# ishine/ASR-Rescoring

Measured on NVIDIA B200. Metric: N-best PLL hypotheses/sec, higher is better.
Workload: dtype bf16+fp16head

## Files before the change

### asr-rescoring_b200/build.py

```python
from __future__ import annotations

import os
import subprocess
import sys

HERE = os.path.dirname(os.path.abspath(__file__))
CSRC = os.path.join(HERE, "csrc")
LIB = os.path.join(HERE, "libpllb200.so")
ARCH = ["-gencode", "arch=compute_100a,code=sm_100a"]
COMMON = ["-O3", "-std=c++17", "-lineinfo", "-Xcompiler", "-fPIC", "-Xcompiler", "-Wall",
          "--expt-relaxed-constexpr", "-Xptxas", "-v"]
UNITS = {
    "api.cu": [],
    "gemm_tcgen05.cu": [],
    "gemm_ln_tcgen05.cu": [],
    "encoder_kernels.cu": [],
    "train_kernels.cu": [],
    "train_api.cu": [],
    "bertscore_kernels.cu": [],
    "seq2seq_kernels.cu": [],
    "seq2seq_api.cu": [],
    "rescore_kernels.cu": ["-fmad=false", "-prec-div=true", "-prec-sqrt=true"],
}


def _nvcc() -> str:
    for cand in (os.environ.get("NVCC"), "/usr/local/cuda/bin/nvcc", "nvcc"):
        if cand and (os.path.isabs(cand) and os.path.exists(cand) or not os.path.isabs(cand)):
            return cand
    raise RuntimeError("nvcc not found")
# ... 61 lines not shown
```

### asr-rescoring_b200/csrc/api.cu

```cuda
#include <cuda_bf16.h>

#include <nvtx3/nvToolsExt.h>

#include <algorithm>
#include <cstdlib>
#include <cstring>
#include <unordered_map>
#include <vector>

#include "common.h"

namespace pllb {

static thread_local std::string g_last_error;
thread_local int64_t g_launch_counter = 0;

void set_error(const std::string& msg) { g_last_error = msg; }
int fail(int code, const std::string& msg) {
  g_last_error = msg;
  return code;
}

int check_model_shape(const pllb_model_desc& d) {
  if (d.hidden % 256 != 0 || d.hidden < 256 || d.hidden > 1024 || d.num_heads * 64 != d.hidden ||
// ... 71 lines not shown
  g_tmaps.emplace(key, *out);
  return PLLB_OK;
}

}

using namespace pllb;

namespace {

enum GemmKind { G_QKV = 0, G_AO, G_FF1, G_FF2, G_HEAD, G_DEC, G_KINDS };

struct LayerDev {
  __nv_bfloat16 *qkv_w, *ao_w, *ff1_w, *ff2_w;
  float *qkv_b, *ao_b, *ao_g, *ao_be, *ff1_b, *ff2_b, *out_g, *out_be;
};

struct ClsHead {
  const float* w;
  float b;
  float* out;
};

struct NvtxRange {
  explicit NvtxRange(const char* name) { nvtxRangePushA(name); }
  void next(const char* name) { nvtxRangePop(); nvtxRangePushA(name); }
  ~NvtxRange() { nvtxRangePop(); }
};

struct TimedLaunch {
  cudaEvent_t start, stop;
// ... 1 lines not shown
};

}

struct pllb_context {
  pllb_model_desc d{};
  int device = 0;
  int fp16_from = 0;
  bool head_fp16 = false;
  int dt_head = DT_BF16;
  bool lfp16(int l) const { return l >= fp16_from; }
  int ldt(int l) const { return lfp16(l) ? DT_FP16 : DT_BF16; }
  int ldt_ffn2(int l, bool next_fp16) const { return lfp16(l) ? DT_FP16 : (next_fp16 ? DT_BF16_OUT16 : DT_BF16); }
  bool has_head = false;
  bool share_l0 = true;
  int64_t cap_rows = 0, cap_copies = 0, cap_hyps = 0;
  int vocab_pad = 0, tiles_v = 0;
  std::vector<void*> owned;
  int64_t owned_bytes = 0;
  float *word_emb = nullptr, *pos_emb = nullptr, *type_emb = nullptr, *emb_g = nullptr, *emb_b = nullptr;
  std::vector<LayerDev> layers;
  __nv_bfloat16 *head_w = nullptr, *dec_w = nullptr;
  float *head_b = nullptr, *head_g = nullptr, *head_be = nullptr, *dec_b = nullptr;
  float *hidden_f32 = nullptr, *y_f32 = nullptr;
  __nv_bfloat16 *hidden_bf16 = nullptr, *wide = nullptr , *ctx = nullptr;
  CopyPlan plan{};
  __nv_bfloat16 *hg = nullptr, *t_bf16 = nullptr;
  float *t_f32 = nullptr, *hid_c = nullptr, *label_logit = nullptr, *tok_logp = nullptr;
  float2* partials = nullptr;
  int32_t* meta_dev = nullptr;
// ... 79 lines not shown
               int K, int epi, const LseArgs* lse, cudaStream_t s, int dt) {
  const double fl = 2.0 * (double)M * (double)(epi == EPI_LSE && lse ? lse->vocab : N) * (double)K;
  return timed_launch(c, kind, fl, s, [&] { return launch_gemm_tcgen05(A, W, bias, C, M, N, K, epi, lse, dt, s); });
}

int timed_gemm_ln(pllb_context* c, int kind, const void* A, const void* W, const float* bias, const float* g,
                  const float* be, float* hid32, void* hid16, int64_t M, int K, cudaStream_t s, int dt) {
  const int H = c->d.hidden;
  const double fl = 2.0 * (double)M * (double)H * (double)K;
  return timed_launch(c, kind, fl, s,
                      [&] { return launch_gemm_ln(A, W, bias, g, be, c->d.ln_eps, hid32, hid16, M, H, K, dt, s); });
}

int run_chunk(pllb_context* c, const int32_t* tokens, const int32_t* tok_off, const int32_t* copy_base,
              const int32_t* row_base, int32_t n_hyp, int32_t n_copies, int64_t n_rows, int max_T, double* out_pll,
              float* out_tok_logp, int upto_layer, cudaStream_t s, const ClsHead* cls = nullptr,
              float* out_cls = nullptr) {
  const pllb_model_desc& d = c->d;
  const int H = d.hidden, I = d.intermediate;
  NvtxRange r_chunk("pllb chunk");
  NvtxRange r_stage("stage1: masked-copy expansion + embeddings");
  RC(launch_expand_plan(tokens, tok_off, copy_base, row_base, n_hyp, d.vocab, cls != nullptr, c->plan, s));
  const int n_layers = upto_layer < 0 ? d.num_layers : std::min(upto_layer, d.num_layers);
  const int64_t n_unique = 2 * (int64_t)n_copies + 2 * (int64_t)n_hyp;
  const bool share = c->share_l0 && !cls && 2 * n_unique <= n_rows;
  if (share) {
    RC(launch_embed_unique(tokens, tok_off, n_hyp, c->word_emb, c->pos_emb, c->type_emb, c->emb_g, c->emb_b, d.ln_eps,
                           H, d.cls_id, d.sep_id, d.mask_id, d.vocab, c->y_f32, c->ctx, c->lfp16(0), s));
    RC(launch_row_src(c->plan, n_copies, s));
    RC(launch_rowmajor_to_t32(c->y_f32, c->plan.row_src, c->hidden_f32, n_rows, H, s));
  } else {
    RC(launch_embed_ln(tokens, tok_off, c->plan, n_copies, c->word_emb, c->pos_emb, c->type_emb, c->emb_g, c->emb_b,
// ... 3 lines not shown
  const bool prune_last = upto_layer < 0 && n_layers > 0;
  r_stage.next("stage2: encoder");
  for (int l = 0; l < n_layers; ++l) {
    const LayerDev& L = c->layers[l];
    const bool shared_rows = share && l == 0;
    const bool last = prune_last && l == n_layers - 1;
    const bool f16 = c->lfp16(l);
    const int dt = c->ldt(l);
    const int dt_ffn2 = c->ldt_ffn2(l, l + 1 < d.num_layers ? c->lfp16(l + 1) : (cls ? f16 : c->head_fp16));
    if (last && !shared_rows) {
      RC(timed_gemm(c, G_QKV, c->hidden_bf16, L.qkv_w + (size_t)H * H, L.qkv_b + H, c->wide, n_rows, 2 * H, H,
                    EPI_BIAS_BF16, nullptr, s, dt));
      RC(launch_gather_rows_bf16(c->hidden_bf16, c->plan.mask_row, n_copies, H, c->hg, s));
      RC(timed_gemm(c, G_QKV, c->hg, L.qkv_w, L.qkv_b, c->t_bf16, n_copies, H, H, EPI_BIAS_BF16, nullptr, s, dt));
      RC(launch_attention_row(c->t_bf16, c->wide, c->hg, c->plan, n_copies, H, d.num_heads, max_T, f16, s));
    } else {
      RC(timed_gemm(c, G_QKV, shared_rows ? c->ctx : c->hidden_bf16, L.qkv_w, L.qkv_b, c->wide,
                    shared_rows ? n_unique : n_rows, 3 * H, H, EPI_BIAS_BF16, nullptr, s, dt));
      RC(launch_attention(c->wide, c->ctx, c->plan, n_copies, H, d.num_heads, f16, shared_rows, s));
      if (last) RC(launch_gather_rows_bf16(c->ctx, c->plan.mask_row, n_copies, H, c->hg, s));
    }
    if (last) {
      RC(launch_gather_rows_f32(c->hidden_f32, c->plan.mask_row, n_copies, H, c->hid_c, s));
      RC(timed_gemm_ln(c, G_AO, c->hg, L.ao_w, L.ao_b, L.ao_g, L.ao_be, c->hid_c, c->t_bf16, n_copies, H, s, dt));
      RC(timed_gemm(c, G_FF1, c->t_bf16, L.ff1_w, L.ff1_b, c->wide, n_copies, I, H, EPI_BIAS_GELU_BF16, nullptr, s, dt));
      RC(timed_gemm_ln(c, G_FF2, c->wide, L.ff2_w, L.ff2_b, L.out_g, L.out_be, c->hid_c, c->t_bf16, n_copies, I, s, dt_ffn2));
      break;
    }
    RC(timed_gemm_ln(c, G_AO, c->ctx, L.ao_w, L.ao_b, L.ao_g, L.ao_be, c->hidden_f32, c->hidden_bf16, n_rows, H, s, dt));
    RC(timed_gemm(c, G_FF1, c->hidden_bf16, L.ff1_w, L.ff1_b, c->wide, n_rows, I, H, EPI_BIAS_GELU_BF16, nullptr, s, dt));
// ... 9 lines not shown
  RC(timed_gemm(c, G_HEAD, c->t_bf16, c->head_w, c->head_b, c->t_f32, n_copies, H, H, EPI_BIAS_GELU_F32, nullptr, s,
                c->dt_head));
  RC(launch_plain_ln_bf16(c->t_f32, c->hg, c->head_g, c->head_be, d.ln_eps, n_copies, H, c->head_fp16, s));
  LseArgs lse{c->plan.label, c->partials, c->label_logit, d.vocab};
  RC(timed_gemm(c, G_DEC, c->hg, c->dec_w, c->dec_b, nullptr, n_copies, c->vocab_pad, H, EPI_LSE, &lse, s, c->dt_head));
  RC(launch_lse_finish(c->partials, c->label_logit, n_copies, 2 * c->tiles_v, c->tok_logp, s));
  RC(launch_hyp_sum(c->tok_logp, copy_base, n_hyp, out_pll, out_tok_logp, s));
  return PLLB_OK;
}

struct Chunk {
  int32_t hyp_begin, n_hyp, n_copies;
  int64_t n_rows, tok_begin;
  int max_T;
  int64_t meta_off;
};

int ensure_meta(pllb_context* c, int64_t need, cudaStream_t s) {
  if (need <= c->meta_cap) return PLLB_OK;
  PLLB_CUDA(cudaStreamSynchronize(s));
  PLLB_CUDA(cudaDeviceSynchronize());
  if (c->meta_dev) cudaFree(c->meta_dev);
  if (c->meta_host) cudaFreeHost(c->meta_host);
  c->meta_dev = nullptr;
  c->meta_host = nullptr;
  const int64_t cap = need + need / 2 + 1024;
  PLLB_CUDA(cudaMalloc(&c->meta_dev, sizeof(int32_t) * cap));
  PLLB_CUDA(cudaHostAlloc(&c->meta_host, sizeof(int32_t) * cap, cudaHostAllocDefault));
  c->meta_cap = cap;
  return PLLB_OK;
}
// ... 26 lines not shown
  c->meta_pending = true;
  return PLLB_OK;
}

int score_impl(pllb_context* c, const int32_t* hyp_tokens, const int64_t* off, int32_t n_hyp, double* out_pll,
               float* out_tok_logp, int upto_layer, float* out_hidden, cudaStream_t s, const ClsHead* cls = nullptr) {
  if (!c) return fail(PLLB_ERR_INVALID, "null handle");
  if (n_hyp < 0 || (n_hyp > 0 && (!off || !hyp_tokens && off[n_hyp] > off[0])))
    return fail(PLLB_ERR_INVALID, "pllb_score: null argument");
  PLLB_CUDA(cudaSetDevice(c->device));
  const int64_t launches_before = g_launch_counter;
  c->stats.last_gemm_launches = 0;
  c->timed_used = 0;
  std::vector<Chunk> chunks;
  {
    Chunk cur{0, 0, 0, 0, n_hyp > 0 ? off[0] : 0, 0, 0};
    for (int32_t h = 0; h < n_hyp; ++h) {
      const int64_t L = off[h + 1] - off[h];
      if (L < 0) return fail(PLLB_ERR_INVALID, "pllb_score: offsets not monotone");
      if (L + 2 > c->d.max_position)
        return fail(PLLB_ERR_TOO_LONG, "hypothesis " + std::to_string(h) + " has " + std::to_string(L) +
                                           " tokens; max_position_embeddings allows " + std::to_string(c->d.max_position - 2));
      const int64_t rows = cls ? L + 2 : L * (L + 2);
      const int64_t copies = cls ? 1 : L;
      if (rows > c->cap_rows || copies > c->cap_copies)
        return fail(PLLB_ERR_OOM, "a single hypothesis exceeds max_chunk_tokens");
      if (cur.n_hyp > 0 && (cur.n_rows + rows > c->cap_rows || cur.n_copies + copies > c->cap_copies || cur.n_hyp + 1 > c->cap_hyps)) {
        chunks.push_back(cur);
        cur = Chunk{h, 0, 0, 0, off[h], 0, 0};
      }
      cur.n_hyp += 1;
      cur.n_copies += (int32_t)copies;
      cur.n_rows += rows;
      cur.max_T = std::max(cur.max_T, (int)L + 2);
    }
    if (cur.n_hyp > 0) chunks.push_back(cur);
  }
  if (upto_layer >= 0 && !cls && chunks.size() > 1) return fail(PLLB_ERR_OOM, "pllb_debug_hidden: input must fit one chunk");
  int64_t meta_need = 0;
  for (auto& ch : chunks) {
    ch.meta_off = meta_need;
    meta_need += 3 * (int64_t)(ch.n_hyp + 1);
  }
  RC(ensure_meta(c, meta_need, s));
  RC(meta_acquire(c));
  RC(workspace_acquire(c, s));
  for (const auto& ch : chunks) {
    int32_t* tok_off = c->meta_host + ch.meta_off;
    int32_t* copy_base = tok_off + (ch.n_hyp + 1);
    int32_t* row_base = copy_base + (ch.n_hyp + 1);
    int64_t t = 0, cb = 0, rb = 0;
    for (int32_t i = 0; i <= ch.n_hyp; ++i) {
      tok_off[i] = (int32_t)t; copy_base[i] = (int32_t)cb; row_base[i] = (int32_t)rb;
      if (i < ch.n_hyp) {
        const int64_t L = off[ch.hyp_begin + i + 1] - off[ch.hyp_begin + i];
        t += L; cb += cls ? 1 : L; rb += cls ? L + 2 : L * (L + 2);
      }
    }
  }
  RC(meta_upload(c, meta_need, s));
  if (c->timing) {
    if (!c->ev_begin) { PLLB_CUDA(cudaEventCreate(&c->ev_begin)); PLLB_CUDA(cudaEventCreate(&c->ev_end)); }
    PLLB_CUDA(cudaEventRecord(c->ev_begin, s));
  }
  int64_t row0 = 0;
  for (const auto& ch : chunks) {
    const int32_t* tok_off = c->meta_dev + ch.meta_off;
    const int32_t* copy_base = tok_off + (ch.n_hyp + 1);
    const int32_t* row_base = copy_base + (ch.n_hyp + 1);
    RC(run_chunk(c, hyp_tokens + (ch.tok_begin - off[0]), tok_off, copy_base, row_base, ch.n_hyp, ch.n_copies, ch.n_rows,
                 ch.max_T, out_pll ? out_pll + ch.hyp_begin : nullptr,
                 out_tok_logp ? out_tok_logp + (ch.tok_begin - off[0]) : nullptr, upto_layer, s, cls,
                 cls && cls->out ? cls->out + ch.hyp_begin : nullptr));
    if (out_hidden) RC(launch_t32_to_rowmajor(c->hidden_f32, out_hidden + row0 * c->d.hidden, ch.n_rows, c->d.hidden, s));
    row0 += ch.n_rows;
    c->stats.chunks += 1;
    c->stats.hyps_scored += ch.n_hyp;
    c->stats.copies_scored += ch.n_copies;
    c->stats.tokens_expanded += ch.n_rows;
  }
  if (c->timing) { PLLB_CUDA(cudaEventRecord(c->ev_end, s)); c->have_total = true; }
  RC(workspace_release(c, s));
  c->stats.kernel_launches += g_launch_counter - launches_before;
  return PLLB_OK;
}

int ensure_io(pllb_context* c, int64_t bytes) {
  if (bytes <= c->io_cap) return PLLB_OK;
// ... 72 lines not shown
  if (d.operand_dtype < 0 || (d.operand_dtype > 3 && (d.operand_dtype < 16 || d.operand_dtype > 16 + d.num_layers)))
    return fail(PLLB_ERR_INVALID, "unsupported model shape: need num_layers >= 1, hidden in {256,512,768,1024}, "
                                  "head dim 64, intermediate % 256 == 0");
  PLLB_CUDA(cudaSetDevice(device));
  int major = 0;
  PLLB_CUDA(cudaDeviceGetAttribute(&major, cudaDevAttrComputeCapabilityMajor, device));
  if (major != 10) return fail(PLLB_ERR_NO_DEVICE, "device is not sm_100 (B200); libpllb200 has no other code path");
  pllb_context* c = new pllb_context();
  c->d = d;
  c->device = device;
  c->fp16_from = d.operand_dtype == 1 ? 0 : d.operand_dtype == 3 ? d.num_layers / 2
               : d.operand_dtype >= 16 ? d.operand_dtype - 16 : d.num_layers;
  c->head_fp16 = d.operand_dtype >= 1;
  c->dt_head = c->head_fp16 ? DT_FP16 : DT_BF16;
  if (const char* e = getenv("PLLB_SHARE_L0")) c->share_l0 = atoi(e) != 0;
  cudaStream_t s = 0;
  const int H = d.hidden, I = d.intermediate, V = d.vocab;
  int rc = PLLB_OK;
  auto bail = [&](int code) {
    pllb_destroy(c);
    return code;
  };
#define TRY(expr)                  \
  do {                             \
    rc = (expr);                   \
    if (rc) return bail(rc);       \
  } while (0)
  TRY(copy_f32(c, &c->word_emb, w->word_emb, (int64_t)V * H, s));
  TRY(copy_f32(c, &c->pos_emb, w->pos_emb, (int64_t)d.max_position * H, s));
  TRY(copy_f32(c, &c->type_emb, w->type_emb, H, s));
  TRY(copy_f32(c, &c->emb_g, w->emb_ln_g, H, s));
  TRY(copy_f32(c, &c->emb_b, w->emb_ln_b, H, s));
  c->layers.resize(d.num_layers);
  for (int l = 0; l < d.num_layers; ++l) {
    const pllb_layer_weights& lw = w->layers[l];
    LayerDev& L = c->layers[l];
    TRY(dev_alloc(c, &L.qkv_w, (int64_t)3 * H * H));
    TRY(launch_f32_to_bf16(lw.q_w, L.qkv_w, (int64_t)H * H, c->lfp16(l), s));
    TRY(launch_f32_to_bf16(lw.k_w, L.qkv_w + (int64_t)H * H, (int64_t)H * H, c->lfp16(l), s));
    TRY(launch_f32_to_bf16(lw.v_w, L.qkv_w + (int64_t)2 * H * H, (int64_t)H * H, c->lfp16(l), s));
    TRY(dev_alloc(c, &L.qkv_b, 3 * H));
    cudaMemcpyAsync(L.qkv_b, lw.q_b, sizeof(float) * H, cudaMemcpyDeviceToDevice, s);
    cudaMemcpyAsync(L.qkv_b + H, lw.k_b, sizeof(float) * H, cudaMemcpyDeviceToDevice, s);
    cudaMemcpyAsync(L.qkv_b + 2 * H, lw.v_b, sizeof(float) * H, cudaMemcpyDeviceToDevice, s);
    TRY(conv_16(c, &L.ao_w, lw.ao_w, (int64_t)H * H, c->lfp16(l), s));
    TRY(copy_f32(c, &L.ao_b, lw.ao_b, H, s));
    TRY(copy_f32(c, &L.ao_g, lw.ao_ln_g, H, s));
    TRY(copy_f32(c, &L.ao_be, lw.ao_ln_b, H, s));
    TRY(conv_16(c, &L.ff1_w, lw.ff1_w, (int64_t)I * H, c->lfp16(l), s));
    TRY(copy_f32(c, &L.ff1_b, lw.ff1_b, I, s));
    TRY(conv_16(c, &L.ff2_w, lw.ff2_w, (int64_t)H * I, c->lfp16(l), s));
    TRY(copy_f32(c, &L.ff2_b, lw.ff2_b, H, s));
    TRY(copy_f32(c, &L.out_g, lw.out_ln_g, H, s));
    TRY(copy_f32(c, &L.out_be, lw.out_ln_b, H, s));
  }
  c->vocab_pad = (int)align_up(V, 256);
  c->tiles_v = c->vocab_pad / 256;
  c->has_head = w->head_w && w->head_b && w->head_ln_g && w->head_ln_b && w->decoder_w && w->decoder_b;
  if (c->has_head) {
// ... 567 lines not shown
```

### asr-rescoring_b200/csrc/common.h

```cpp
#pragma once
#include <cuda.h>
#include <cuda_runtime.h>
#include <stdint.h>

#include <cstdio>
#include <string>
#include <utility>
#include <vector>

#include "../../include/pllb.h"

namespace pllb {

void set_error(const std::string& msg);
int fail(int code, const std::string& msg);
extern thread_local int64_t g_launch_counter;
__attribute__((visibility("hidden"))) int check_model_shape(const pllb_model_desc& d);

#define PLLB_CUDA(expr)                                                                        \
  do {                                                                                         \
    cudaError_t _e = (expr);                                                                   \
    if (_e != cudaSuccess)                                                                     \
      return ::pllb::fail(PLLB_ERR_CUDA, std::string(#expr) + ": " + cudaGetErrorString(_e));  \
  } while (0)
// ... 74 lines not shown

int launch_expand_plan(const int32_t* tokens, const int32_t* hyp_tok_off, const int32_t* hyp_copy_base,
                       const int32_t* hyp_row_base, int32_t n_hyp, int32_t vocab, bool whole_sequence, CopyPlan plan,
                       cudaStream_t s);
int launch_expand_ids(const int32_t* tokens, const int32_t* hyp_tok_off, CopyPlan plan, int32_t n_copies,
                      int32_t cls_id, int32_t sep_id, int32_t mask_id, int32_t* out_ids, int32_t* out_mask_pos,
                      int32_t* out_labels, cudaStream_t s);
int launch_embed_ln(const int32_t* tokens, const int32_t* hyp_tok_off, CopyPlan plan, int32_t n_copies,
                    const float* word_emb, const float* pos_emb, const float* type_emb, const float* g,
                    const float* b, float eps, int H, int32_t cls_id, int32_t sep_id, int32_t mask_id, int32_t vocab,
                    float* hidden_f32_rowmajor, void* hidden_bf16, bool fp16, cudaStream_t s);
int launch_plain_ln_bf16(const float* x, void* out_bf16, const float* g, const float* b, float eps, int64_t rows,
                         int H, bool fp16, cudaStream_t s);
int launch_attention(const void* qkv_bf16, void* ctx_bf16, CopyPlan plan, int32_t n_copies, int H, int NH, bool fp16,
                     bool shared_rows, cudaStream_t s);
int launch_embed_unique(const int32_t* tokens, const int32_t* hyp_tok_off, int32_t n_hyp, const float* word_emb,
                        const float* pos_emb, const float* type_emb, const float* g, const float* b, float eps, int H,
                        int32_t cls_id, int32_t sep_id, int32_t mask_id, int32_t vocab, float* u_f32, void* u_bf16,
                        bool fp16, cudaStream_t s);
int launch_row_src(CopyPlan plan, int32_t n_copies, cudaStream_t s);
int launch_attention_row(const void* q_bf16, const void* kv_bf16, void* out_bf16, CopyPlan plan, int32_t n_copies, int H,
                         int NH, int max_T, bool fp16, cudaStream_t s);
int launch_gather_rows_bf16(const void* hidden_bf16, const int32_t* rows, int32_t n, int H, void* out,
                            cudaStream_t s);
int launch_gather_rows_f32(const float* src, const int32_t* rows, int32_t n, int H, float* out, cudaStream_t s);
int launch_cls_linear(const float* hid_t32, const float* w, float b, int32_t n, int H, float* out, cudaStream_t s);
int launch_lse_finish(const float2* partials, const float* label_logit, int32_t n_copies, int n_tiles,
                      float* tok_logp, cudaStream_t s);
int launch_hyp_sum(const float* tok_logp, const int32_t* hyp_copy_base, int32_t n_hyp, double* out_pll,
                   float* out_tok_logp, cudaStream_t s);
// ... 65 lines not shown
```

### asr-rescoring_b200/csrc/encoder_kernels.cu

```cuda
#include <cuda_bf16.h>
#include <cuda_fp16.h>

#include "common.h"
#include "ptx.cuh"

namespace pllb {

namespace {

constexpr int WARPS_PER_BLOCK = 8;

__device__ __forceinline__ float warp_sum(float v) {
#pragma unroll
  for (int o = 16; o > 0; o >>= 1) v += __shfl_xor_sync(0xffffffffu, v, o);
  return v;
}
__device__ __forceinline__ float warp_max(float v) {
#pragma unroll
  for (int o = 16; o > 0; o >>= 1) v = fmaxf(v, __shfl_xor_sync(0xffffffffu, v, o));
  return v;
}

template <bool FP16>
__device__ __forceinline__ uint32_t pack16(float lo, float hi) {
// ... 181 lines not shown
          const float* __restrict__ b, float eps, int64_t rows) {
  constexpr int H = 128 * VEC;
  const int64_t row = (int64_t)blockIdx.x * WARPS_PER_BLOCK + (threadIdx.x >> 5);
  const int lane = threadIdx.x & 31;
  if (row >= rows) return;
  const float4* yr = reinterpret_cast<const float4*>(y + row * H);
  float4 x[VEC];
#pragma unroll
  for (int i = 0; i < VEC; ++i) x[i] = yr[lane + 32 * i];
  ln_normalize<VEC>(x, g, b, eps, lane);
  store_row<VEC, FP16>(x, out_bf16 + row * H, lane);
}

constexpr int ATT_WARPS = 8;
constexpr int ATT_VROW = 72;

__device__ __forceinline__ float fast_ex2(float x) {
  float y;
  asm("ex2.approx.ftz.f32 %0, %1;" : "=f"(y) : "f"(x));
  return y;
}

template <bool FP16>
__device__ __forceinline__ void mma_16816(float (&d)[4], const uint32_t (&a)[4], uint32_t b0, uint32_t b1) {
  if constexpr (FP16) {
    asm volatile(
        "mma.sync.aligned.m16n8k16.row.col.f32.f16.f16.f32 {%0,%1,%2,%3}, {%4,%5,%6,%7}, {%8,%9}, {%0,%1,%2,%3};"
        : "+f"(d[0]), "+f"(d[1]), "+f"(d[2]), "+f"(d[3])
        : "r"(a[0]), "r"(a[1]), "r"(a[2]), "r"(a[3]), "r"(b0), "r"(b1));
  } else {
    asm volatile(
        "mma.sync.aligned.m16n8k16.row.col.f32.bf16.bf16.f32 {%0,%1,%2,%3}, {%4,%5,%6,%7}, {%8,%9}, {%0,%1,%2,%3};"
        : "+f"(d[0]), "+f"(d[1]), "+f"(d[2]), "+f"(d[3])
        : "r"(a[0]), "r"(a[1]), "r"(a[2]), "r"(a[3]), "r"(b0), "r"(b1));
  }
}

struct RowDirect {
  size_t start_ld, ld;
  __device__ __forceinline__ size_t operator()(int r) const { return start_ld + (size_t)r * ld; }
};
struct RowShared {
  int ubase, umask, mpos;
  size_t ld;
  __device__ __forceinline__ size_t operator()(int r) const { return (size_t)(r == mpos ? umask : ubase + r) * ld; }
};

template <bool FP16, class RM>
__device__ __forceinline__ void attn_stream(const __nv_bfloat16* __restrict__ base , const RM rm,
                                            __nv_bfloat16* __restrict__ ob, int T, int H, int lane, __nv_bfloat16* vs) {
  const __nv_bfloat16* kb = base + H;
// ... 715 lines not shown
```

### asr-rescoring_b200/csrc/ptx.cuh

```cuda
#pragma once
#include <cuda.h>
#include <cuda_runtime.h>
#include <stdint.h>

namespace pllb {

__device__ __forceinline__ uint32_t smem_u32(const void* p) {
  return static_cast<uint32_t>(__cvta_generic_to_shared(p));
}

__device__ __forceinline__ bool elect_one() {
  uint32_t pred = 0;
  asm volatile(
      "{\n\t.reg .pred P;\n\t"
      "elect.sync _|P, 0xffffffff;\n\t"
      "selp.b32 %0, 1, 0, P;\n\t}\n"
      : "=r"(pred));
  return pred != 0;
}

template <bool FP16>
__device__ __forceinline__ uint32_t pack16x2_sat(float lo, float hi) {
  uint32_t r;
  if constexpr (FP16) asm("cvt.rn.satfinite.f16x2.f32 %0, %1, %2;" : "=r"(r) : "f"(hi), "f"(lo));
// ... 148 lines not shown
}

__device__ __forceinline__ void tmem_ld_32x32b_x32(uint32_t taddr, uint32_t (&r)[32]) {
  asm volatile(
      "tcgen05.ld.sync.aligned.32x32b.x32.b32 "
      "{%0, %1, %2, %3, %4, %5, %6, %7, %8, %9, %10, %11, %12, %13, %14, %15, "
      "%16, %17, %18, %19, %20, %21, %22, %23, %24, %25, %26, %27, %28, %29, %30, %31}, [%32];"
      : "=r"(r[0]), "=r"(r[1]), "=r"(r[2]), "=r"(r[3]), "=r"(r[4]), "=r"(r[5]), "=r"(r[6]), "=r"(r[7]),
        "=r"(r[8]), "=r"(r[9]), "=r"(r[10]), "=r"(r[11]), "=r"(r[12]), "=r"(r[13]), "=r"(r[14]), "=r"(r[15]),
        "=r"(r[16]), "=r"(r[17]), "=r"(r[18]), "=r"(r[19]), "=r"(r[20]), "=r"(r[21]), "=r"(r[22]), "=r"(r[23]),
        "=r"(r[24]), "=r"(r[25]), "=r"(r[26]), "=r"(r[27]), "=r"(r[28]), "=r"(r[29]), "=r"(r[30]), "=r"(r[31])
      : "r"(taddr)
      : "memory");
}

__device__ __forceinline__ float2 ffma2(float2 a, float2 b, float2 c) {
  float2 d;
  asm("{.reg .b64 ra, rb, rc, rd;\n\t"
      "mov.b64 ra, {%2,%3};\n\t mov.b64 rb, {%4,%5};\n\t mov.b64 rc, {%6,%7};\n\t"
      "fma.rn.f32x2 rd, ra, rb, rc;\n\t mov.b64 {%0,%1}, rd;}"
      : "=f"(d.x), "=f"(d.y) : "f"(a.x), "f"(a.y), "f"(b.x), "f"(b.y), "f"(c.x), "f"(c.y));
  return d;
}
__device__ __forceinline__ float2 fmul2(float2 a, float2 b) {
  float2 d;
  asm("{.reg .b64 ra, rb, rd;\n\t"
      "mov.b64 ra, {%2,%3};\n\t mov.b64 rb, {%4,%5};\n\t"
      "mul.rn.f32x2 rd, ra, rb;\n\t mov.b64 {%0,%1}, rd;}"
      : "=f"(d.x), "=f"(d.y) : "f"(a.x), "f"(a.y), "f"(b.x), "f"(b.y));
  return d;
}
__device__ __forceinline__ float2 fadd2(float2 a, float2 b) {
  float2 d;
  asm("{.reg .b64 ra, rb, rd;\n\t"
      "mov.b64 ra, {%2,%3};\n\t mov.b64 rb, {%4,%5};\n\t"
      "add.rn.f32x2 rd, ra, rb;\n\t mov.b64 {%0,%1}, rd;}"
      : "=f"(d.x), "=f"(d.y) : "f"(a.x), "f"(a.y), "f"(b.x), "f"(b.y));
  return d;
}

__device__ __forceinline__ uint64_t make_kmajor_sw128_desc(uint32_t smem_addr) {
  uint64_t d = 0;
  d |= (uint64_t)((smem_addr & 0x3FFFF) >> 4);
  d |= (uint64_t)1 << 16;
  d |= (uint64_t)(1024 >> 4) << 32;
  d |= (uint64_t)1 << 46;
  d |= (uint64_t)2 << 61;
  return d;
}
__host__ __device__ constexpr uint32_t make_idesc_bf16(int M, int N) {
  return (1u << 4) | (1u << 7) | (1u << 10) | ((uint32_t)(N >> 3) << 17) | ((uint32_t)(M >> 4) << 24);
}
__host__ __device__ constexpr uint32_t make_idesc_f16(int M, int N) {
// ... 9 lines not shown
```

Before: 20760.

## Fuse QKV projection GEMM with per-copy attention in a 2-CTA tcgen05 kernel

Adds a new kernel that computes the QKV projection per head on tcgen05 tensor cores (2-CTA clusters, interleaved per-head QKV weights), stages Q/K/V tiles in shared memory and runs flash-style attention with mma.sync directly from them, writing only the context. Masked copies are packed into 128-row runs on the host so each tile holds whole sequences. The path is used when max_T fits a run and padding overhead stays under 15%. This removes the wide QKV buffer round-trip through global memory and a separate attention launch. The cost is extra weight memory for the interleaved copies, padded rows in runs, and heavier epilogue warps.

Result: no change. 20870, median of 6 (+0.6%).

```diff
diff --git a/asr-rescoring_b200/build.py b/asr-rescoring_b200/build.py
--- a/asr-rescoring_b200/build.py
+++ b/asr-rescoring_b200/build.py
@@ -14,6 +14,7 @@
     "api.cu": [],
     "gemm_tcgen05.cu": [],
     "gemm_ln_tcgen05.cu": [],
+    "fused_attention_tcgen05.cu": [],
     "encoder_kernels.cu": [],
     "train_kernels.cu": [],
     "train_api.cu": [],
diff --git a/asr-rescoring_b200/csrc/api.cu b/asr-rescoring_b200/csrc/api.cu
--- a/asr-rescoring_b200/csrc/api.cu
+++ b/asr-rescoring_b200/csrc/api.cu
@@ -109,7 +109,12 @@
 struct LayerDev {
   __nv_bfloat16 *qkv_w, *ao_w, *ff1_w, *ff2_w;
   float *qkv_b, *ao_b, *ao_g, *ao_be, *ff1_b, *ff2_b, *out_g, *out_be;
+  __nv_bfloat16* qkv_wi = nullptr;
+  float* qkv_bi = nullptr;
 };
+
+constexpr double kFuseMaxPadding = 0.15;
+constexpr int kRunRows = 128;
 
 struct ClsHead {
   const float* w;
@@ -141,6 +146,7 @@
   int ldt_ffn2(int l, bool next_fp16) const { return lfp16(l) ? DT_FP16 : (next_fp16 ? DT_BF16_OUT16 : DT_BF16); }
   bool has_head = false;
   bool share_l0 = true;
+  bool fuse_att = true;
   int64_t cap_rows = 0, cap_copies = 0, cap_hyps = 0;
   int vocab_pad = 0, tiles_v = 0;
   std::vector<void*> owned;
@@ -250,8 +256,8 @@
 
 int run_chunk(pllb_context* c, const int32_t* tokens, const int32_t* tok_off, const int32_t* copy_base,
               const int32_t* row_base, int32_t n_hyp, int32_t n_copies, int64_t n_rows, int max_T, double* out_pll,
-              float* out_tok_logp, int upto_layer, cudaStream_t s, const ClsHead* cls = nullptr,
-              float* out_cls = nullptr) {
+              float* out_tok_logp, int upto_layer, cudaStream_t s, const int32_t* run_copy, int32_t n_runs,
+              const ClsHead* cls = nullptr, float* out_cls = nullptr) {
   const pllb_model_desc& d = c->d;
   const int H = d.hidden, I = d.intermediate;
   NvtxRange r_chunk("pllb chunk");
@@ -285,6 +291,11 @@
       RC(launch_gather_rows_bf16(c->hidden_bf16, c->plan.mask_row, n_copies, H, c->hg, s));
       RC(timed_gemm(c, G_QKV, c->hg, L.qkv_w, L.qkv_b, c->t_bf16, n_copies, H, H, EPI_BIAS_BF16, nullptr, s, dt));
       RC(launch_attention_row(c->t_bf16, c->wide, c->hg, c->plan, n_copies, H, d.num_heads, max_T, f16, s));
+    } else if (n_runs > 0 && !shared_rows) {
+      RC(timed_launch(c, G_QKV, 2.0 * (double)n_rows * 3 * H * H, s, [&] {
+        return launch_fused_qkv_attention(c->hidden_bf16, L.qkv_wi, L.qkv_bi, c->ctx, n_rows, H, d.num_heads, run_copy,
+                                          n_runs, c->plan, f16, s);
+      }));
     } else {
       RC(timed_gemm(c, G_QKV, shared_rows ? c->ctx : c->hidden_bf16, L.qkv_w, L.qkv_b, c->wide,
                     shared_rows ? n_unique : n_rows, 3 * H, H, EPI_BIAS_BF16, nullptr, s, dt));
@@ -324,7 +335,26 @@
   int64_t n_rows, tok_begin;
   int max_T;
   int64_t meta_off;
+  int32_t n_runs;
 };
+
+int32_t plan_runs(const int64_t* off, int32_t hyp_begin, int32_t n_hyp, int32_t* run_copy) {
+  int32_t n_runs = 0, copy = 0;
+  int64_t used = kRunRows;
+  for (int32_t h = hyp_begin; h < hyp_begin + n_hyp; ++h) {
+    const int64_t L = off[h + 1] - off[h], T = L + 2;
+    for (int64_t m = 0; m < L; ++m, ++copy) {
+      if (used + T > kRunRows) {
+        if (run_copy) run_copy[n_runs] = copy;
+        ++n_runs;
+        used = 0;
+      }
+      used += T;
+    }
+  }
+  if (run_copy) run_copy[n_runs] = copy;
+  return n_runs;
+}
 
 int ensure_meta(pllb_context* c, int64_t need, cudaStream_t s) {
   if (need <= c->meta_cap) return PLLB_OK;
@@ -381,7 +411,7 @@
   c->timed_used = 0;
   std::vector<Chunk> chunks;
   {
-    Chunk cur{0, 0, 0, 0, n_hyp > 0 ? off[0] : 0, 0, 0};
+    Chunk cur{0, 0, 0, 0, n_hyp > 0 ? off[0] : 0, 0, 0, 0};
     for (int32_t h = 0; h < n_hyp; ++h) {
       const int64_t L = off[h + 1] - off[h];
       if (L < 0) return fail(PLLB_ERR_INVALID, "pllb_score: offsets not monotone");
@@ -394,7 +424,7 @@
         return fail(PLLB_ERR_OOM, "a single hypothesis exceeds max_chunk_tokens");
       if (cur.n_hyp > 0 && (cur.n_rows + rows > c->cap_rows || cur.n_copies + copies > c->cap_copies || cur.n_hyp + 1 > c->cap_hyps)) {
         chunks.push_back(cur);
-        cur = Chunk{h, 0, 0, 0, off[h], 0, 0};
+        cur = Chunk{h, 0, 0, 0, off[h], 0, 0, 0};
       }
       cur.n_hyp += 1;
       cur.n_copies += (int32_t)copies;
@@ -408,6 +438,13 @@
   for (auto& ch : chunks) {
     ch.meta_off = meta_need;
     meta_need += 3 * (int64_t)(ch.n_hyp + 1);
+    if (c->fuse_att && !cls && ch.max_T <= kRunRows && ch.n_copies > 0) {
+      const int32_t n_runs = plan_runs(off, ch.hyp_begin, ch.n_hyp, nullptr);
+      if ((double)n_runs * kRunRows < (1.0 + kFuseMaxPadding) * (double)ch.n_rows) {
+        ch.n_runs = n_runs;
+        meta_need += n_runs + 1;
+      }
+    }
   }
   RC(ensure_meta(c, meta_need, s));
   RC(meta_acquire(c));
@@ -424,6 +461,7 @@
         t += L; cb += cls ? 1 : L; rb += cls ? L + 2 : L * (L + 2);
       }
     }
+    if (ch.n_runs > 0) plan_runs(off, ch.hyp_begin, ch.n_hyp, row_base + (ch.n_hyp + 1));
   }
   RC(meta_upload(c, meta_need, s));
   if (c->timing) {
@@ -437,8 +475,8 @@
     const int32_t* row_base = copy_base + (ch.n_hyp + 1);
     RC(run_chunk(c, hyp_tokens + (ch.tok_begin - off[0]), tok_off, copy_base, row_base, ch.n_hyp, ch.n_copies, ch.n_rows,
                  ch.max_T, out_pll ? out_pll + ch.hyp_begin : nullptr,
-                 out_tok_logp ? out_tok_logp + (ch.tok_begin - off[0]) : nullptr, upto_layer, s, cls,
-                 cls && cls->out ? cls->out + ch.hyp_begin : nullptr));
+                 out_tok_logp ? out_tok_logp + (ch.tok_begin - off[0]) : nullptr, upto_layer, s,
+                 row_base + (ch.n_hyp + 1), ch.n_runs, cls, cls && cls->out ? cls->out + ch.hyp_begin : nullptr));
     if (out_hidden) RC(launch_t32_to_rowmajor(c->hidden_f32, out_hidden + row0 * c->d.hidden, ch.n_rows, c->d.hidden, s));
     row0 += ch.n_rows;
     c->stats.chunks += 1;
@@ -541,6 +579,7 @@
   c->head_fp16 = d.operand_dtype >= 1;
   c->dt_head = c->head_fp16 ? DT_FP16 : DT_BF16;
   if (const char* e = getenv("PLLB_SHARE_L0")) c->share_l0 = atoi(e) != 0;
+  if (const char* e = getenv("PLLB_FUSE_ATT")) c->fuse_att = atoi(e) != 0;
   cudaStream_t s = 0;
   const int H = d.hidden, I = d.intermediate, V = d.vocab;
   int rc = PLLB_OK;
@@ -570,6 +609,18 @@
     cudaMemcpyAsync(L.qkv_b, lw.q_b, sizeof(float) * H, cudaMemcpyDeviceToDevice, s);
     cudaMemcpyAsync(L.qkv_b + H, lw.k_b, sizeof(float) * H, cudaMemcpyDeviceToDevice, s);
     cudaMemcpyAsync(L.qkv_b + 2 * H, lw.v_b, sizeof(float) * H, cudaMemcpyDeviceToDevice, s);
+    if (c->fuse_att) {
+      TRY(dev_alloc(c, &L.qkv_wi, (int64_t)3 * H * H));
+      TRY(dev_alloc(c, &L.qkv_bi, 3 * H));
+      for (int h = 0; h < d.num_heads; ++h)
+        for (int part = 0; part < 3; ++part) {
+          const int64_t src = (int64_t)part * H + h * 64, dst = (int64_t)h * 192 + part * 64;
+          TRY(cudaMemcpyAsync(L.qkv_wi + dst * H, L.qkv_w + src * H, sizeof(__nv_bfloat16) * 64 * H,
+                              cudaMemcpyDeviceToDevice, s) == cudaSuccess ? PLLB_OK : fail(PLLB_ERR_CUDA, "qkv interleave"));
+          TRY(cudaMemcpyAsync(L.qkv_bi + dst, L.qkv_b + src, sizeof(float) * 64, cudaMemcpyDeviceToDevice, s) == cudaSuccess
+                  ? PLLB_OK : fail(PLLB_ERR_CUDA, "qkv interleave"));
+        }
+    }
     TRY(conv_16(c, &L.ao_w, lw.ao_w, (int64_t)H * H, c->lfp16(l), s));
     TRY(copy_f32(c, &L.ao_b, lw.ao_b, H, s));
     TRY(copy_f32(c, &L.ao_g, lw.ao_ln_g, H, s));
diff --git a/asr-rescoring_b200/csrc/common.h b/asr-rescoring_b200/csrc/common.h
--- a/asr-rescoring_b200/csrc/common.h
+++ b/asr-rescoring_b200/csrc/common.h
@@ -112,6 +112,9 @@
                          int H, bool fp16, cudaStream_t s);
 int launch_attention(const void* qkv_bf16, void* ctx_bf16, CopyPlan plan, int32_t n_copies, int H, int NH, bool fp16,
                      bool shared_rows, cudaStream_t s);
+int launch_fused_qkv_attention(const void* A, const void* W_il, const float* bias_il, void* ctx, int64_t rows, int H,
+                               int NH, const int32_t* run_copy, int32_t n_runs, CopyPlan plan, bool fp16,
+                               cudaStream_t stream);
 int launch_embed_unique(const int32_t* tokens, const int32_t* hyp_tok_off, int32_t n_hyp, const float* word_emb,
                         const float* pos_emb, const float* type_emb, const float* g, const float* b, float eps, int H,
                         int32_t cls_id, int32_t sep_id, int32_t mask_id, int32_t vocab, float* u_f32, void* u_bf16,
diff --git a/asr-rescoring_b200/csrc/encoder_kernels.cu b/asr-rescoring_b200/csrc/encoder_kernels.cu
--- a/asr-rescoring_b200/csrc/encoder_kernels.cu
+++ b/asr-rescoring_b200/csrc/encoder_kernels.cu
@@ -219,27 +219,6 @@
 
 constexpr int ATT_WARPS = 8;
 constexpr int ATT_VROW = 72;
-
-__device__ __forceinline__ float fast_ex2(float x) {
-  float y;
-  asm("ex2.approx.ftz.f32 %0, %1;" : "=f"(y) : "f"(x));
-  return y;
-}
-
-template <bool FP16>
-__device__ __forceinline__ void mma_16816(float (&d)[4], const uint32_t (&a)[4], uint32_t b0, uint32_t b1) {
-  if constexpr (FP16) {
-    asm volatile(
-        "mma.sync.aligned.m16n8k16.row.col.f32.f16.f16.f32 {%0,%1,%2,%3}, {%4,%5,%6,%7}, {%8,%9}, {%0,%1,%2,%3};"
-        : "+f"(d[0]), "+f"(d[1]), "+f"(d[2]), "+f"(d[3])
-        : "r"(a[0]), "r"(a[1]), "r"(a[2]), "r"(a[3]), "r"(b0), "r"(b1));
-  } else {
-    asm volatile(
-        "mma.sync.aligned.m16n8k16.row.col.f32.bf16.bf16.f32 {%0,%1,%2,%3}, {%4,%5,%6,%7}, {%8,%9}, {%0,%1,%2,%3};"
-        : "+f"(d[0]), "+f"(d[1]), "+f"(d[2]), "+f"(d[3])
-        : "r"(a[0]), "r"(a[1]), "r"(a[2]), "r"(a[3]), "r"(b0), "r"(b1));
-  }
-}
 
 struct RowDirect {
   size_t start_ld, ld;
diff --git a/asr-rescoring_b200/csrc/fused_attention_tcgen05.cu b/asr-rescoring_b200/csrc/fused_attention_tcgen05.cu
--- /dev/null
+++ b/asr-rescoring_b200/csrc/fused_attention_tcgen05.cu
@@ -0,0 +1,392 @@
+#include <cuda_bf16.h>
+#include <cuda_fp16.h>
+
+#include <algorithm>
+
+#include "common.h"
+#include "ptx.cuh"
+
+namespace pllb {
+
+namespace {
+
+constexpr int FA_BM = 128;
+constexpr int FA_BN = 192;
+constexpr int FA_BK = 64;
+constexpr int FA_UMMA_K = 16;
+constexpr int FA_STAGES = 4;
+constexpr int FA_A_BYTES = FA_BM * FA_BK * 2;
+constexpr int FA_B_BYTES = (FA_BN / 2) * FA_BK * 2;
+constexpr int FA_EPI_WARPS = 14;
+constexpr int FA_STAGE_WARPS = 12;
+constexpr int FA_WARP_COLS = FA_BN / (FA_STAGE_WARPS / 4);
+constexpr int FA_LD_COLS = 32;
+constexpr int FA_THREADS = 32 * (2 + FA_EPI_WARPS);
+static_assert(FA_WARP_COLS % FA_LD_COLS == 0 && 64 % FA_LD_COLS == 0, "staging chunks");
+constexpr int FA_ACC_STRIDE = 256;
+constexpr int FA_TMEM_COLS = 512;
+constexpr int FA_VROW = 72;
+constexpr int FA_SROWS = FA_BM + 16;
+constexpr int FA_MAT_BYTES = FA_SROWS * FA_VROW * 2;
+constexpr int FA_OUT_BYTES = 16 * FA_VROW * 2;
+constexpr int FA_PIPE = FA_STAGES * (FA_A_BYTES + FA_B_BYTES);
+constexpr int FA_SMEM_STAGE = 3 * FA_MAT_BYTES;
+constexpr int FA_SMEM_OUT = FA_EPI_WARPS * FA_OUT_BYTES;
+constexpr int FA_SMEM_BARS = 256;
+constexpr int FA_SMEM_TOTAL = FA_PIPE + FA_SMEM_STAGE + FA_SMEM_OUT + FA_SMEM_BARS + 1024;
+static_assert(FA_SMEM_TOTAL <= 227 * 1024, "shared memory budget");
+
+struct FaParams {
+  const int32_t* run_copy;
+  int32_t n_runs;
+  const int32_t* seq_start;
+  const int32_t* seq_len;
+  const float* bias;
+  __nv_bfloat16* ctx;
+  int H, NH;
+};
+
+__device__ __forceinline__ void epi_bar(int id) {
+  asm volatile("bar.sync %0, %1;" ::"r"(id), "n"(FA_EPI_WARPS * 32) : "memory");
+}
+
+template <bool FP16>
+__device__ __forceinline__ void attend_block(uint32_t q_addr, uint32_t k_addr, uint32_t v_addr, int m0, int T,
+                                             __nv_bfloat16* __restrict__ ob, int H, int lane, uint32_t out_addr,
+                                             const __nv_bfloat16* out_sm) {
+  const int g = lane >> 2, cq = lane & 3;
+  constexpr float kScaleLog2 = 0.125f * 1.4426950408889634f;
+  const int lrow = (lane & 7) + ((lane >> 3) & 1) * 8, lcol8 = ((lane >> 4) & 1) * 8;
+  uint32_t qf[4][4];
+#pragma unroll
+  for (int ks = 0; ks < 4; ++ks) {
+    const uint32_t addr = q_addr + (uint32_t)((m0 + lrow) * FA_VROW + 16 * ks + lcol8) * 2;
+    asm volatile("ldmatrix.sync.aligned.m8n8.x4.shared.b16 {%0,%1,%2,%3}, [%4];"
+                 : "=r"(qf[ks][0]), "=r"(qf[ks][1]), "=r"(qf[ks][2]), "=r"(qf[ks][3]) : "r"(addr));
+  }
+  float mx[2] = {-INFINITY, -INFINITY}, l[2] = {0.f, 0.f};
+  float o[8][4];
+#pragma unroll
+  for (int n = 0; n < 8; ++n) { o[n][0] = o[n][1] = o[n][2] = o[n][3] = 0.f; }
+  for (int k0 = 0; k0 < T; k0 += 16) {
+    float s[2][4];
+#pragma unroll
+    for (int j = 0; j < 2; ++j) {
+      s[j][0] = s[j][1] = s[j][2] = s[j][3] = 0.f;
+      if (j == 1 && k0 + 8 >= T) break;
+#pragma unroll
+      for (int kp = 0; kp < 2; ++kp) {
+        const uint32_t addr = k_addr + (uint32_t)((k0 + 8 * j + (lane & 7)) * FA_VROW + 32 * kp + (lane >> 3) * 8) * 2;
+        uint32_t b0, b1, b2, b3;
+        asm volatile("ldmatrix.sync.aligned.m8n8.x4.shared.b16 {%0,%1,%2,%3}, [%4];"
+                     : "=r"(b0), "=r"(b1), "=r"(b2), "=r"(b3) : "r"(addr));
+        mma_16816<FP16>(s[j], qf[2 * kp], b0, b1);
+        mma_16816<FP16>(s[j], qf[2 * kp + 1], b2, b3);
+      }
+    }
+    float bm[2] = {-INFINITY, -INFINITY};
+    const bool tail = k0 + 16 > T;
+#pragma unroll
+    for (int j = 0; j < 2; ++j) {
+#pragma unroll
+      for (int e = 0; e < 4; ++e) {
+        const int key = k0 + 8 * j + 2 * cq + (e & 1);
+        s[j][e] = (!tail || key < T) ? s[j][e] * kScaleLog2 : -INFINITY;
+        bm[e >> 1] = fmaxf(bm[e >> 1], s[j][e]);
+      }
+    }
+    float corr[2];
+#pragma unroll
+    for (int r = 0; r < 2; ++r) {
+      bm[r] = fmaxf(bm[r], __shfl_xor_sync(0xffffffffu, bm[r], 1));
+      bm[r] = fmaxf(bm[r], __shfl_xor_sync(0xffffffffu, bm[r], 2));
+      const float nm = fmaxf(mx[r], bm[r]);
+      corr[r] = fast_ex2(mx[r] - nm);
+      mx[r] = nm;
+      l[r] *= corr[r];
+    }
+    uint32_t pf[4];
+    {
+      const float p00 = fast_ex2(s[0][0] - mx[0]), p01 = fast_ex2(s[0][1] - mx[0]);
+      const float p02 = fast_ex2(s[0][2] - mx[1]), p03 = fast_ex2(s[0][3] - mx[1]);
+      const float p10 = fast_ex2(s[1][0] - mx[0]), p11 = fast_ex2(s[1][1] - mx[0]);
+      const float p12 = fast_ex2(s[1][2] - mx[1]), p13 = fast_ex2(s[1][3] - mx[1]);
+      l[0] += (p00 + p01) + (p10 + p11);
+      l[1] += (p02 + p03) + (p12 + p13);
+      pf[0] = pack16x2_sat<FP16>(p00, p01); pf[1] = pack16x2_sat<FP16>(p02, p03);
+      pf[2] = pack16x2_sat<FP16>(p10, p11); pf[3] = pack16x2_sat<FP16>(p12, p13);
+    }
+    if (k0 > 0) {
+#pragma unroll
+      for (int n = 0; n < 8; ++n) {
+        o[n][0] *= corr[0]; o[n][1] *= corr[0]; o[n][2] *= corr[1]; o[n][3] *= corr[1];
+      }
+    }
+#pragma unroll
+    for (int n = 0; n < 8; n += 2) {
+      const uint32_t addr = v_addr + (uint32_t)((k0 + lrow) * FA_VROW + 8 * n + lcol8) * 2;
+      uint32_t b0, b1, b2, b3;
+      asm volatile("ldmatrix.sync.aligned.m8n8.x4.trans.shared.b16 {%0,%1,%2,%3}, [%4];"
+                   : "=r"(b0), "=r"(b1), "=r"(b2), "=r"(b3) : "r"(addr));
+      mma_16816<FP16>(o[n], pf, b0, b1);
+      mma_16816<FP16>(o[n + 1], pf, b2, b3);
+    }
+  }
+#pragma unroll
+  for (int r = 0; r < 2; ++r) {
+    l[r] += __shfl_xor_sync(0xffffffffu, l[r], 1);
+    l[r] += __shfl_xor_sync(0xffffffffu, l[r], 2);
+  }
+  const float inv0 = 1.0f / l[0], inv1 = 1.0f / l[1];
+  __syncwarp();
+  {
+    const uint32_t st0 = out_addr + (uint32_t)(g * FA_VROW + 2 * cq) * 2, st1 = st0 + 8 * FA_VROW * 2;
+#pragma unroll
+    for (int n = 0; n < 8; ++n) {
+      asm volatile("st.shared.b32 [%0], %1;" ::"r"(st0 + 16 * n), "r"(pack16x2_sat<FP16>(o[n][0] * inv0, o[n][1] * inv0)) : "memory");
+      asm volatile("st.shared.b32 [%0], %1;" ::"r"(st1 + 16 * n), "r"(pack16x2_sat<FP16>(o[n][2] * inv1, o[n][3] * inv1)) : "memory");
+    }
+  }
+  __syncwarp();
+  {
+    const int r_off = lane >> 3, ch = lane & 7;
+#pragma unroll
+    for (int rr = 0; rr < 16; rr += 4) {
+      const int q = m0 + rr + r_off;
+      if (q < T)
+        *reinterpret_cast<uint4*>(ob + (size_t)q * H + ch * 8) =
+            *reinterpret_cast<const uint4*>(out_sm + (rr + r_off) * FA_VROW + ch * 8);
+    }
+  }
+}
+
+template <bool FP16>
+__global__ void __launch_bounds__(FA_THREADS, 1)
+fused_qkv_attention_kernel(const __grid_constant__ CUtensorMap tmA, const __grid_constant__ CUtensorMap tmB,
+                           const FaParams p) {
+  extern __shared__ uint8_t smem_raw[];
+  const uint32_t smem_base = (smem_u32(smem_raw) + 1023u) & ~1023u;
+  uint8_t* smem_gen = smem_raw + (smem_base - smem_u32(smem_raw));
+  const uint32_t sA = smem_base;
+  const uint32_t sB = smem_base + FA_STAGES * FA_A_BYTES;
+  const uint32_t sQ = smem_base + FA_PIPE;
+  const uint32_t sOut = sQ + FA_SMEM_STAGE;
+  const uint32_t sBar = sOut + FA_SMEM_OUT;
+  const uint32_t bar_full = sBar;
+  const uint32_t bar_empty = sBar + 8 * FA_STAGES;
+  const uint32_t bar_tfull = sBar + 16 * FA_STAGES;
+  const uint32_t bar_tempty = bar_tfull + 16;
+  const uint32_t tmem_slot = bar_tempty + 16;
+  uint32_t* tmem_slot_ptr = reinterpret_cast<uint32_t*>(smem_gen + (tmem_slot - smem_base));
+
+  const int warp = threadIdx.x >> 5;
+  const int lane = threadIdx.x & 31;
+  const int num_kb = p.H / FA_BK;
+  const uint32_t crank = cluster_ctarank();
+  const int unit0 = (int)(blockIdx.x >> 1);
+  const int unit_stride = (int)(gridDim.x >> 1);
+  const int num_tiles = ((p.n_runs + 1) / 2) * p.NH;
+
+  if (warp == 0 && lane == 0) {
+    prefetch_tensormap(&tmA);
+    prefetch_tensormap(&tmB);
+  }
+  if (warp == 1) {
+    if (lane == 0) {
+      for (int s = 0; s < FA_STAGES; ++s) {
+        mbar_init(bar_full + 8 * s, 1);
+        mbar_init(bar_empty + 8 * s, 1);
+      }
+      for (int s = 0; s < 2; ++s) {
+        mbar_init(bar_tfull + 8 * s, 1);
+        mbar_init(bar_tempty + 8 * s, 2 * FA_STAGE_WARPS);
+      }
+      fence_barrier_init();
+    }
+    __syncwarp();
+    tmem_alloc_2cta(tmem_slot, FA_TMEM_COLS);
+    tmem_relinquish_2cta();
+  }
+  if (warp >= 2) {
+    const int t = threadIdx.x - 64;
+    for (int i = t; i < 3 * 16 * FA_VROW / 8; i += FA_EPI_WARPS * 32) {
+      const int mat = i / (16 * FA_VROW / 8), e = i % (16 * FA_VROW / 8);
+      *reinterpret_cast<uint4*>(smem_gen + FA_PIPE + mat * FA_MAT_BYTES + FA_BM * FA_VROW * 2 + e * 16) =
+          make_uint4(0, 0, 0, 0);
+    }
+  }
+  tcgen05_fence_before();
+  __syncthreads();
+  cluster_sync_all();
+  tcgen05_fence_after();
+  const uint32_t tmem_base = *tmem_slot_ptr;
+
+  if (warp == 0) {
+    if (lane == 0) {
+      uint32_t stage = 0, phase = 0;
+      auto first_row = [&](int tile) {
+        const int run = 2 * (tile / p.NH) + (int)crank;
+        return tile < num_tiles && run < p.n_runs ? p.seq_start[p.run_copy[run]] : 0;
+      };
+      int next_row0 = first_row(unit0);
+      for (int tile = unit0; tile < num_tiles; tile += unit_stride) {
+        const int head = tile % p.NH;
+        const int row0 = next_row0;
+        next_row0 = first_row(tile + unit_stride);
+        for (int kb = 0; kb < num_kb; ++kb) {
+          mbar_wait(bar_empty + 8 * stage, phase ^ 1);
+          const uint32_t lead_full = mapa_shared(bar_full + 8 * stage, 0);
+          if (crank == 0) mbar_arrive_expect_tx(bar_full + 8 * stage, 2 * (FA_A_BYTES + FA_B_BYTES));
+          tma_load_2d_2sm(sA + stage * FA_A_BYTES, &tmA, lead_full, kb * FA_BK, row0);
+          tma_load_2d_2sm(sB + stage * FA_B_BYTES, &tmB, lead_full, kb * FA_BK, head * FA_BN + (int)crank * (FA_BN / 2));
+          if (++stage == FA_STAGES) { stage = 0; phase ^= 1; }
+        }
+      }
+    }
+  } else if (warp == 1) {
+    if (lane == 0 && crank == 0) {
+      constexpr uint32_t idesc = make_idesc_16(2 * FA_BM, FA_BN, FP16, FP16);
+      uint32_t stage = 0, phase = 0, acc = 0, acc_phase = 0;
+      for (int tile = unit0; tile < num_tiles; tile += unit_stride) {
+        mbar_wait(bar_tempty + 8 * acc, acc_phase ^ 1);
+        tcgen05_fence_after();
+        const uint32_t d_tmem = tmem_base + acc * FA_ACC_STRIDE;
+        for (int kb = 0; kb < num_kb; ++kb) {
+          mbar_wait(bar_full + 8 * stage, phase);
+          tcgen05_fence_after();
+          const uint32_t a_addr = sA + stage * FA_A_BYTES;
+          const uint32_t b_addr = sB + stage * FA_B_BYTES;
+#pragma unroll
+          for (int k = 0; k < FA_BK / FA_UMMA_K; ++k) {
+            const uint64_t adesc = make_kmajor_sw128_desc(a_addr + k * FA_UMMA_K * 2);
+            const uint64_t bdesc = make_kmajor_sw128_desc(b_addr + k * FA_UMMA_K * 2);
+            tcgen05_mma_bf16_2cta(d_tmem, adesc, bdesc, idesc, (kb | k) != 0 ? 1u : 0u);
+          }
+          tcgen05_commit_2cta_multicast(bar_empty + 8 * stage, (uint16_t)0x3);
+          if (++stage == FA_STAGES) { stage = 0; phase ^= 1; }
+        }
+        tcgen05_commit_2cta_multicast(bar_tfull + 8 * acc, (uint16_t)0x3);
+        acc ^= 1;
+        if (acc == 0) acc_phase ^= 1;
+      }
+    }
+  } else {
+    const int q = warp & 3;
+    const int ew = warp - 2;
+    const int cbase = (ew >> 2) * FA_WARP_COLS;
+    const int srow = q * 32 + lane;
+    const uint32_t out_addr = sOut + ew * FA_OUT_BYTES;
+    const __nv_bfloat16* out_sm = reinterpret_cast<const __nv_bfloat16*>(smem_gen + FA_PIPE + FA_SMEM_STAGE + ew * FA_OUT_BYTES);
+    uint32_t acc = 0, acc_phase = 0;
+    for (int tile = unit0; tile < num_tiles; tile += unit_stride) {
+      const int run = 2 * (tile / p.NH) + (int)crank;
+      const int head = tile % p.NH;
+      int n_cp = 0, st_a = 0, t_a = 0, st_b = 0, t_b = 0;
+      if (run < p.n_runs) {
+        const int c_begin = p.run_copy[run];
+        n_cp = p.run_copy[run + 1] - c_begin;
+        if (lane < n_cp) { st_a = p.seq_start[c_begin + lane]; t_a = p.seq_len[c_begin + lane]; }
+        if (lane + 32 < n_cp) { st_b = p.seq_start[c_begin + 32 + lane]; t_b = p.seq_len[c_begin + 32 + lane]; }
+      }
+      mbar_wait(bar_tfull + 8 * acc, acc_phase);
+      tcgen05_fence_after();
+      epi_bar(1);
+      const uint32_t t_addr = tmem_base + acc * FA_ACC_STRIDE + ((uint32_t)(q * 32) << 16);
+      const float* bias = p.bias + head * FA_BN;
+#pragma unroll
+      for (int ci = 0; ci < (ew < FA_STAGE_WARPS ? FA_WARP_COLS / FA_LD_COLS : 0); ++ci) {
+        const int c0 = cbase + FA_LD_COLS * ci;
+        uint32_t r[FA_LD_COLS];
+        tmem_ld_32x32b_x32(t_addr + c0, r);
+        tcgen05_wait_ld();
+        if (ci == FA_WARP_COLS / FA_LD_COLS - 1) {
+          tcgen05_fence_before();
+          __syncwarp();
+          if (lane == 0) mbar_arrive_cluster(mapa_shared(bar_tempty + 8 * acc, 0));
+        }
+        const uint32_t dst = sQ + (uint32_t)(c0 >> 6) * FA_MAT_BYTES + (uint32_t)(srow * FA_VROW + (c0 & 63)) * 2;
+        const float4* bias4 = reinterpret_cast<const float4*>(bias + c0);
+#pragma unroll
+        for (int c = 0; c < FA_LD_COLS / 8; ++c) {
+          const float4 b0 = __ldg(bias4 + 2 * c), b1 = __ldg(bias4 + 2 * c + 1);
+          const float2 v0 = fadd2(make_float2(__uint_as_float(r[8 * c + 0]), __uint_as_float(r[8 * c + 1])), make_float2(b0.x, b0.y));
+          const float2 v1 = fadd2(make_float2(__uint_as_float(r[8 * c + 2]), __uint_as_float(r[8 * c + 3])), make_float2(b0.z, b0.w));
+          const float2 v2 = fadd2(make_float2(__uint_as_float(r[8 * c + 4]), __uint_as_float(r[8 * c + 5])), make_float2(b1.x, b1.y));
+          const float2 v3 = fadd2(make_float2(__uint_as_float(r[8 * c + 6]), __uint_as_float(r[8 * c + 7])), make_float2(b1.z, b1.w));
+          asm volatile("st.shared.v4.b32 [%0], {%1, %2, %3, %4};" ::"r"(dst + 16 * c),
+                       "r"(pack16x2_sat<FP16>(v0.x, v0.y)), "r"(pack16x2_sat<FP16>(v1.x, v1.y)),
+                       "r"(pack16x2_sat<FP16>(v2.x, v2.y)), "r"(pack16x2_sat<FP16>(v3.x, v3.y))
+                       : "memory");
+        }
+      }
+      acc ^= 1;
+      if (acc == 0) acc_phase ^= 1;
+      epi_bar(2);
+      {
+        const int row0 = __shfl_sync(0xffffffffu, st_a, 0);
+        int unit = 0;
+        for (int i = 0; i < n_cp; ++i) {
+          const int start = __shfl_sync(0xffffffffu, i < 32 ? st_a : st_b, i & 31);
+          const int T = __shfl_sync(0xffffffffu, i < 32 ? t_a : t_b, i & 31);
+          const uint32_t off = (uint32_t)((start - row0) * FA_VROW) * 2;
+          __nv_bfloat16* ob = p.ctx + (size_t)start * p.H + head * 64;
+          for (int m0 = 0; m0 < T; m0 += 16, ++unit) {
+            if (unit % FA_EPI_WARPS != ew) continue;
+            attend_block<FP16>(sQ + off, sQ + FA_MAT_BYTES + off, sQ + 2 * FA_MAT_BYTES + off, m0, T, ob, p.H, lane,
+                               out_addr, out_sm);
+          }
+        }
+      }
+    }
+  }
+
+  tcgen05_fence_before();
+  __syncthreads();
+  cluster_sync_all();
+  if (warp == 1) {
+    __syncwarp();
+    tcgen05_fence_after();
+    tmem_dealloc_2cta(tmem_base, FA_TMEM_COLS);
+  }
+}
+
+}
+
+int launch_fused_qkv_attention(const void* A, const void* W_il, const float* bias_il, void* ctx, int64_t rows, int H,
+                               int NH, const int32_t* run_copy, int32_t n_runs, CopyPlan plan, bool fp16,
+                               cudaStream_t stream) {
+  if (n_runs <= 0) return PLLB_OK;
+  if (H != NH * 64 || H % FA_BK != 0 || rows > INT32_MAX)
+    return fail(PLLB_ERR_INVALID, "fused attention: need head dim 64 and H % 64 == 0");
+  CUtensorMap ta, tb;
+  int rc;
+  if ((rc = get_tmap_2d(&ta, A, CU_TENSOR_MAP_DATA_TYPE_BFLOAT16, 2, (uint64_t)rows, (uint64_t)H, FA_BM, FA_BK))) return rc;
+  if ((rc = get_tmap_2d(&tb, W_il, CU_TENSOR_MAP_DATA_TYPE_BFLOAT16, 2, (uint64_t)3 * H, (uint64_t)H, FA_BN / 2, FA_BK)))
+    return rc;
+  FaParams fp{run_copy, n_runs, plan.seq_start, plan.seq_len, bias_il, reinterpret_cast<__nv_bfloat16*>(ctx), H, NH};
+  const int64_t tiles = (int64_t)((n_runs + 1) / 2) * NH;
+  const int64_t clusters = std::min<int64_t>(tiles, sm_count() / 2);
+  cudaLaunchConfig_t cfg{};
+  cfg.gridDim = dim3((unsigned)(2 * clusters));
+  cfg.blockDim = dim3(FA_THREADS);
+  cfg.dynamicSmemBytes = FA_SMEM_TOTAL;
+  cfg.stream = stream;
+  cudaLaunchAttribute attr[1];
+  attr[0].id = cudaLaunchAttributeClusterDimension;
+  attr[0].val.clusterDim.x = 2;
+  attr[0].val.clusterDim.y = 1;
+  attr[0].val.clusterDim.z = 1;
+  cfg.attrs = attr;
+  cfg.numAttrs = 1;
+  if (fp16) {
+    PLLB_CUDA(opt_in_smem(fused_qkv_attention_kernel<true>, FA_SMEM_TOTAL));
+    PLLB_CUDA(cudaLaunchKernelEx(&cfg, fused_qkv_attention_kernel<true>, ta, tb, fp));
+  } else {
+    PLLB_CUDA(opt_in_smem(fused_qkv_attention_kernel<false>, FA_SMEM_TOTAL));
+    PLLB_CUDA(cudaLaunchKernelEx(&cfg, fused_qkv_attention_kernel<false>, ta, tb, fp));
+  }
+  ++g_launch_counter;
+  return PLLB_OK;
+}
+
+}
diff --git a/asr-rescoring_b200/csrc/ptx.cuh b/asr-rescoring_b200/csrc/ptx.cuh
--- a/asr-rescoring_b200/csrc/ptx.cuh
+++ b/asr-rescoring_b200/csrc/ptx.cuh
@@ -186,6 +186,16 @@
       : "memory");
 }
 
+__device__ __forceinline__ void tmem_ld_32x32b_x16(uint32_t taddr, uint32_t (&r)[16]) {
+  asm volatile(
+      "tcgen05.ld.sync.aligned.32x32b.x16.b32 "
+      "{%0, %1, %2, %3, %4, %5, %6, %7, %8, %9, %10, %11, %12, %13, %14, %15}, [%16];"
+      : "=r"(r[0]), "=r"(r[1]), "=r"(r[2]), "=r"(r[3]), "=r"(r[4]), "=r"(r[5]), "=r"(r[6]), "=r"(r[7]),
+        "=r"(r[8]), "=r"(r[9]), "=r"(r[10]), "=r"(r[11]), "=r"(r[12]), "=r"(r[13]), "=r"(r[14]), "=r"(r[15])
+      : "r"(taddr)
+      : "memory");
+}
+
 __device__ __forceinline__ float2 ffma2(float2 a, float2 b, float2 c) {
   float2 d;
   asm("{.reg .b64 ra, rb, rc, rd;\n\t"
@@ -209,6 +219,27 @@
       "add.rn.f32x2 rd, ra, rb;\n\t mov.b64 {%0,%1}, rd;}"
       : "=f"(d.x), "=f"(d.y) : "f"(a.x), "f"(a.y), "f"(b.x), "f"(b.y));
   return d;
+}
+
+__device__ __forceinline__ float fast_ex2(float x) {
+  float y;
+  asm("ex2.approx.ftz.f32 %0, %1;" : "=f"(y) : "f"(x));
+  return y;
+}
+
+template <bool FP16>
+__device__ __forceinline__ void mma_16816(float (&d)[4], const uint32_t (&a)[4], uint32_t b0, uint32_t b1) {
+  if constexpr (FP16) {
+    asm volatile(
+        "mma.sync.aligned.m16n8k16.row.col.f32.f16.f16.f32 {%0,%1,%2,%3}, {%4,%5,%6,%7}, {%8,%9}, {%0,%1,%2,%3};"
+        : "+f"(d[0]), "+f"(d[1]), "+f"(d[2]), "+f"(d[3])
+        : "r"(a[0]), "r"(a[1]), "r"(a[2]), "r"(a[3]), "r"(b0), "r"(b1));
+  } else {
+    asm volatile(
+        "mma.sync.aligned.m16n8k16.row.col.f32.bf16.bf16.f32 {%0,%1,%2,%3}, {%4,%5,%6,%7}, {%8,%9}, {%0,%1,%2,%3};"
+        : "+f"(d[0]), "+f"(d[1]), "+f"(d[2]), "+f"(d[3])
+        : "r"(a[0]), "r"(a[1]), "r"(a[2]), "r"(a[3]), "r"(b0), "r"(b1));
+  }
 }
 
 __device__ __forceinline__ uint64_t make_kmajor_sw128_desc(uint32_t smem_addr) {
```
